# HSU-ANT/gstpeaq

Measured on AMD Instinct MI355X. Metric: 2048-sample stereo ref/test frame-pairs/sec (basic PEAQ, ear model -> MOVs -> ODG); ODG delta vs CPU ref, higher is better.
Workload: dtype f64

## Files before the change

### gstpeaq_amd/capi.py

```python
import ctypes as C
import os
import subprocess
from pathlib import Path

import numpy as np

PKG = Path(__file__).resolve().parent
ROOT = PKG.parent

MOV_NAMES_BASIC = ["BandwidthRefB", "BandwidthTestB", "TotalNMRB", "WinModDiff1B", "ADBB", "EHSB",
                   "AvgModDiff1B", "AvgModDiff2B", "RmsNoiseLoudB", "MFPDB", "RelDistFramesB"]
MOV_NAMES_ADVANCED = ["RmsModDiffA", "RmsNoiseLoudAsymA", "SegmentalNMRB", "EHSB", "AvgLinDistA"]

RESULT_DOUBLES = 16
RECORD_DOUBLES = 576


class Settings(C.Structure):
    _fields_ = [("swap_mod_patts_for_noise_loudness_movs", C.c_int), ("center_ehs_correlation_window", C.c_int),
                ("ehs_subtract_dc_before_window", C.c_int), ("use_floor_for_steps_above_threshold", C.c_int),
                ("clamp_movs", C.c_int), ("swap_slope_filter_coefficients", C.c_int)]


class PeaqError(RuntimeError):
# ... 197 lines not shown
        L.peaq_batch_measure_gain.argtypes = [vp, C.c_int, C.c_int, vp, C.c_size_t, u32p, vp, C.c_size_t, u32p, u32p, C.c_int,
                                              C.c_double, vp, vp]
        L.peaq_gain_workspace_bytes.restype = C.c_size_t
        L.peaq_gain_workspace_bytes.argtypes = [C.c_int, C.c_int, C.c_uint32]
        L.peaq_batch_cut_scaled.argtypes = [vp, C.c_int, C.c_int, vp, C.c_size_t, u32p, u32p, vp, vp, C.c_size_t, vp]
        L.peaq_run_pair_matched.argtypes = [vp, C.c_int, C.c_int, C.c_double, C.c_uint32, C.c_uint32, C.c_int, C.c_double, fp,
                                            C.c_size_t, fp, C.c_size_t, C.POINTER(Delay), C.POINTER(Gain), dp]
        L.peaq_batch_run_host_matched.argtypes = [vp, C.c_int, C.c_double, C.POINTER(Feed), C.c_int, C.c_double, C.c_size_t,
                                                  C.POINTER(HostSignal), C.c_size_t, C.POINTER(HostTest), dp, C.POINTER(Delay),
                                                  C.POINTER(Gain)]
        L.peaq_feed_matched_workspace_bytes.restype = C.c_size_t
        L.peaq_feed_matched_workspace_bytes.argtypes = [C.POINTER(Feed), C.c_int, C.c_int, C.c_size_t, C.c_size_t, C.c_uint64]
    L.peaq_batch_last_timing.argtypes = [vp, C.POINTER(_Timing)]
    if hasattr(L, "peaq_calibrate"):
        L.peaq_calibrate.argtypes = [vp, C.c_int, C.POINTER(_Calibration)]
        L.peaq_batch_last_clock.argtypes = [vp, dp]
    L.peaq_synth_fill.argtypes = [vp, C.c_uint32, C.c_int, C.c_int, C.c_uint32, C.c_size_t, vp, vp, vp]
    L.peaq_debug_frontend.argtypes = [vp, C.c_int, C.c_int, C.c_double, vp, vp, C.c_uint32, C.c_uint32,
                                      C.c_int, dp]
    L.peaq_debug_filterbank.argtypes = [vp, C.c_int, C.c_double, vp, vp, C.c_uint32, C.c_uint32, C.c_int, C.c_int, dp]
    if hasattr(L, "peaq_debug_wave"):
        L.peaq_debug_wave.argtypes = [vp, C.c_char_p, C.c_size_t, C.c_int, dp, C.c_int, dp, C.c_int, dp]
        L.peaq_debug_common_tables.argtypes = [dp, dp]
    ip = C.POINTER(C.c_int)
    L.peaq_broker_create.argtypes = [vp, C.c_int, C.c_int, C.c_double, C.c_int, C.POINTER(vp)]
    L.peaq_broker_create_multi.argtypes = [C.POINTER(C.c_int), C.c_int, C.c_int, C.c_int, C.c_double, C.c_int, vp, C.c_int,
                                           C.POINTER(vp)]
    L.peaq_broker_devices.argtypes = [vp]
    if hasattr(L, "peaq_debug_broker_fail_shard"):
        L.peaq_debug_broker_fail_shard.argtypes = [vp, C.c_int, C.c_char_p]
    L.peaq_broker_stats_size.argtypes = []
    L.peaq_broker_stats_size.restype = C.c_size_t
    L.peaq_broker_destroy.argtypes = [vp]
    L.peaq_broker_destroy.restype = None
    L.peaq_broker_open.argtypes = [vp, ip]
    L.peaq_broker_close.argtypes = [vp, C.c_int]
    L.peaq_broker_push.argtypes = [vp, C.c_int, C.c_int, fp, C.c_size_t]
    L.peaq_broker_flush.argtypes = [vp, C.c_int]
    L.peaq_broker_tick.argtypes = [vp, C.POINTER(C.c_uint)]
    L.peaq_broker_results.argtypes = [vp, C.c_int, dp]
    L.peaq_broker_start.argtypes = [vp, C.c_uint]
    L.peaq_broker_stop.argtypes = [vp]
    L.peaq_broker_stats.argtypes = [vp, C.POINTER(_BrokerStats)]
    _LIB = L
    return L

# ... 979 lines not shown
```

### gstpeaq_amd/csrc/peaq_debug_wave.hip

```cpp
#include "peaq_host.h"
#include "peaq_wave.h"

using namespace peaq;

namespace {

constexpr int kWgThreads = 256;

enum WaveOp : int {
  OP_LOG_POS, OP_LOG_POS_SK, OP_LOG_NONNEG, OP_LOG_NONNEG_SK, OP_LOG_TAB, OP_LOG_TAB_NONNEG,
  OP_EXP_FAST, OP_EXP_FAST_SK, OP_EXP_TAB, OP_SQRT_POS, OP_RSQRT_POS, OP_DIV_FAST, OP_POW_POS, OP_POW_TAB,
  OP_POW_LOGTAB, OP_LOG_NONNEG_N5, OP_EXP_FAST_N5,
  OP_WAVE_SUM, OP_WAVE_MAX, OP_WAVE_SUM2, OP_WAVE_SUM4, OP_WAVE_PREFIX_SUM, OP_WAVE_SUFFIX_GEOMETRIC,
  OP_WAVE_PREFIX_GEOMETRIC, OP_WAVE_PREFIX_GEOMETRIC_Z, OP_WAVE_PREFIX_GEOMETRIC_F32, OP_ROWS_TRANSPOSE4,
  OP_LANE_BELOW, OP_LANE_ABOVE, OP_READ_LANE_0, OP_READ_LANE_63, OP_DFT4, OP_DFT8, OP_DFT16, OP_COUNT
};

struct OpInfo {
  const char* name;
  int planes_in, planes_out, n_params;
};
const OpInfo kOps[OP_COUNT] = {
    {"log_pos", 1, 1, 0},
    {"log_pos_sk", 1, 1, 0},
// ... 174 lines not shown
                                  " planes and returns " + std::to_string(info.planes_out));
  if (n_params != info.n_params || (n_params > 0 && !params))
    return fail(PEAQ_ERR_ARG, std::string("peaq_debug_wave: ") + op + " takes " + std::to_string(info.n_params) + " parameters");
  if (!c || !in || !out) return fail(PEAQ_ERR_ARG, "peaq_debug_wave: NULL argument");
  if (n > ((size_t)1 << 26)) return fail(PEAQ_ERR_ARG, "peaq_debug_wave: more than 2^26 elements per plane");
  if (n == 0) return PEAQ_OK;
  HIP_TRY(hipSetDevice(c->device));
  const size_t n_pad = (n + kWgThreads - 1) / kWgThreads * kWgThreads;
  DevBuf d_in, d_out;
  HIP_TRY(d_in.reserve((size_t)planes_in * n_pad * sizeof(double)));
  HIP_TRY(d_out.reserve((size_t)planes_out * n_pad * sizeof(double)));
  HIP_TRY(hipMemset(d_in.p, 0, (size_t)planes_in * n_pad * sizeof(double)));
  HIP_TRY(hipMemset(d_out.p, 0, (size_t)planes_out * n_pad * sizeof(double)));
  for (int p = 0; p < planes_in; ++p)
    HIP_TRY(hipMemcpy(d_in.as<double>() + (size_t)p * n_pad, in + (size_t)p * n, n * sizeof(double), hipMemcpyHostToDevice));
  HIP_TRY(hipDeviceSynchronize());
  HIP_TRY(launch_one<0>(which, d_in.as<double>(), d_out.as<double>(), n_pad, n_params ? params[0] : 0., c->d_common));
  HIP_TRY(hipDeviceSynchronize());
  for (int p = 0; p < planes_out; ++p)
    HIP_TRY(hipMemcpy(out + (size_t)p * n, d_out.as<double>() + (size_t)p * n_pad, n * sizeof(double), hipMemcpyDeviceToHost));
  return PEAQ_OK;
}

extern "C" int peaq_debug_common_tables(double* log_tab, double* exp_tab) {
  if (!log_tab || !exp_tab) return fail(PEAQ_ERR_ARG, "peaq_debug_common_tables: NULL argument");
  auto ct = std::make_unique<CommonTables>();
  build_common_tables(*ct);
  std::memcpy(log_tab, ct->log_tab, sizeof ct->log_tab);
  std::memcpy(exp_tab, ct->exp_tab, sizeof ct->exp_tab);
  return PEAQ_OK;
}
```

### gstpeaq_amd/csrc/peaq_frontend.hip

```cpp
#include <hip/hip_runtime.h>

#include "peaq_device.h"
#include "peaq_kernels.h"
#include <type_traits>

#include "peaq_wave.h"

namespace peaq {

#ifndef PEAQ_FE_PREFETCH_ITEMS
#define PEAQ_FE_PREFETCH_ITEMS 64
#endif
constexpr int kPrefetchItems = PEAQ_FE_PREFETCH_ITEMS;
constexpr int kUnitDoubles = 1288;
constexpr int kOffPw = 0;
constexpr int kOffScratch = 776;
constexpr int kPwLen = 776;
constexpr int kOffLogTab = 2 * kUnitDoubles;
constexpr int kLogTabDoubles = 2 * kLogTabEntries + 2;
constexpr int kLdsDoubles = 2 * kUnitDoubles + 2 * kLogTabDoubles;
#ifndef PEAQ_FE_WAVES
#define PEAQ_FE_WAVES 3
#endif
constexpr int kWavesPerSimd = PEAQ_FE_WAVES;

__device__ constexpr double kW32re[16] = {1., 0.98078528040323044913, 0.92387953251128675613, 0.83146961230254523708,
                                          0.70710678118654752440, 0.55557023301960222474, 0.38268343236508977173,
                                          0.19509032201612826785, 0., -0.19509032201612826785, -0.38268343236508977173,
                                          -0.55557023301960222474, -0.70710678118654752440, -0.83146961230254523708,
                                          -0.92387953251128675613, -0.98078528040323044913};
__device__ constexpr double kW32im[16] = {-0., -0.19509032201612826785, -0.38268343236508977173, -0.55557023301960222474,
                                          -0.70710678118654752440, -0.83146961230254523708, -0.92387953251128675613,
                                          -0.98078528040323044913, -1., -0.98078528040323044913, -0.92387953251128675613,
                                          -0.83146961230254523708, -0.70710678118654752440, -0.55557023301960222474,
                                          -0.38268343236508977173, -0.19509032201612826785};

__device__ __forceinline__ int pad16(int i) { return i + (i >> 4); }

__device__ __forceinline__ cplx tw_lane(const CommonTables* __restrict__ ct, int e, int lane) {
  const double2 v = *reinterpret_cast<const double2*>(ct->tw_lane[e][lane]);
  return {v.x, v.y};
}
__device__ __forceinline__ cplx csqr(cplx a) { return {a.re * a.re - a.im * a.im, 2. * (a.re * a.im)}; }

template <typename WR, typename RD>
__device__ __forceinline__ void exchange16(cplx (&z)[16], double* buf, WR wr, RD rd) {
#pragma unroll
  for (int r = 0; r < 16; ++r) buf[pad16(wr(r))] = z[r].re;
  wave_lds_fence();
#pragma unroll
  for (int r = 0; r < 16; ++r) z[r].re = buf[pad16(rd(r))];
  wave_lds_fence();
#pragma unroll
  for (int r = 0; r < 16; ++r) buf[pad16(wr(r))] = z[r].im;
  wave_lds_fence();
#pragma unroll
  for (int r = 0; r < 16; ++r) z[r].im = buf[pad16(rd(r))];
  wave_lds_fence();
}

__device__ __forceinline__ void frame_power_spectrum(cplx (&z)[16], double (&p)[16], double* unit, int lane,
                                                     const CommonTables* __restrict__ ct,
                                                     double level_factor) {
  dft16(z);
// ... 31 lines not shown
        z[4 * a2 + g] = z[4 * g + a2];
        z[4 * g + a2] = t;
      }
#else
    const int k = lane & 15, j = (lane - k) * 16 + k;
    exchange16(z, unit, [&](int r) { return j + 16 * r; },
               [&](int s) { return lane + 64 * (s & 3) + 256 * (s >> 2); });
#endif
  }
  {
    constexpr double c1 = 0.92387953251128673848, s1 = 0.38268343236508977173, c2 = 0.70710678118654752440;
    const cplx wb = tw_lane(ct, 1, lane);
#pragma unroll
    for (int m = 0; m < 4; ++m) {
      const cplx w1 = m == 0 ? wb : m == 1 ? cmul(wb, {c1, -s1}) : m == 2 ? cmul(wb, {c2, -c2}) : cmul(wb, {s1, -c1});
      const cplx w2 = csqr(w1), w3 = cmul(w2, w1);
      z[m + 4] = cmul(z[m + 4], w1);
      z[m + 8] = cmul(z[m + 8], w2);
      z[m + 12] = cmul(z[m + 12], w3);
      dft4(z[m], z[m + 4], z[m + 8], z[m + 12]);
    }
  }
  wave_lds_fence();
  const cplx wl = tw_lane(ct, 0, lane);
  const int partner = (64 - lane) & 63;
  const double lf4 = 0.25 * level_factor;
#pragma unroll
  for (int q = 0; q < 8; ++q) {
    const int k = lane + 64 * q;
    cplx zm = {__shfl(z[15 - q].re, partner, 64), __shfl(z[15 - q].im, partner, 64)};
    if (lane == 0) zm = z[(16 - q) & 15];
    const cplx e2 = {z[q].re + zm.re, z[q].im - zm.im};
    const cplx o2 = {z[q].im + zm.im, zm.re - z[q].re};
    const cplx wq = {kW32re[q], kW32im[q]};
    const cplx t = cmul(q == 0 ? wl : cmul(wl, wq), o2);
    const cplx xp = cadd(e2, t), xm = csub(e2, t);
    p[q] = (xp.re * xp.re + xp.im * xp.im) * lf4;
    double pm = (xm.re * xm.re + xm.im * xm.im) * lf4;
    int km = 1024 - k;
    if (q == 0 && lane == 0) {
      pm = (z[8].re * z[8].re + z[8].im * z[8].im) * level_factor;
      km = 512;
    }
    p[8 + q] = pm;
    const double2 ew = *reinterpret_cast<const double2*>(ct->ear_w2_pair[q][lane]);
    unit[kOffPw + k] = p[q] * ew.x;
    if (km < kPwLen) unit[kOffPw + km] = pm * ew.y;
  }
  wave_lds_fence();
}

__device__ __forceinline__ int spec_bin(int s, int lane) {
  if (s < 8) return lane + 64 * s;
// ... 93 lines not shown
  do {                                                                                 \
    const unsigned long long now_ = __builtin_readcyclecounter();                      \
    if (a.prof && lane == 0 && (blockIdx.x & 127) == 5) atomicAdd(a.prof + sig * 16 + (i), now_ - prof_t_); \
    prof_t_ = __builtin_readcyclecounter();                                            \
  } while (0)
#else
#define FE_MARK(i) do { } while (0)
#endif

template <int NB>
__global__ __launch_bounds__(128, kWavesPerSimd)
#ifdef PEAQ_FE_NUM_VGPR
__attribute__((amdgpu_num_vgpr(PEAQ_FE_NUM_VGPR)))
#endif
void frontend_kernel(FrontendArgs a) {
  extern __shared__ double lds[];
  __builtin_amdgcn_s_setprio(3);
#ifndef PEAQ_FE_LAZY_KERNARGS
  asm volatile("" ::"s"(a.ref), "s"(a.test), "s"(a.pair_stride), "s"(a.n_ref), "s"(a.n_test), "s"(a.n_uniform_ref),
               "s"(a.n_uniform_test), "s"(a.n_frames), "s"(a.n_frames_uniform), "s"(a.frame_origin), "s"(a.off_ref),
               "s"(a.off_test), "s"(a.channels), "s"(a.frame0), "s"(a.frames_per_launch), "s"(a.fpl_magic), "s"(a.common),
               "s"(a.records), "s"(a.pair_frame0), "s"(gridDim.x));
#endif
  const int lane = threadIdx.x & 63;
  const int sig = __builtin_amdgcn_readfirstlane(threadIdx.x >> 6);
#ifdef PEAQ_FE_PROFILE
  unsigned long long prof_t_ = __builtin_readcyclecounter();
  if (a.prof && lane == 0 && (blockIdx.x & 127) == 5) atomicAdd(a.prof + 32 + sig, 1ull);
#endif
  double* unit = lds + sig * kUnitDoubles;
  double* scratch = unit + kOffScratch;
  const CommonTables* __restrict__ ct = a.common;
  const BandTables* __restrict__ bt = a.bands;

  auto decode = [&](unsigned it, unsigned& pair_, unsigned& fl_) {
    const unsigned t = it >> (a.channels - 1);
    pair_ = a.frames_per_launch == 1 ? t : __umulhi(t, a.fpl_magic);
    fl_ = t - pair_ * a.frames_per_launch;
    return (int)(it & (unsigned)(a.channels - 1));
  };
  const unsigned item = xcd_remap(blockIdx.x, gridDim.x);
  unsigned pair, fl;
  const int chan = decode(item, pair, fl);
  FE_MARK(15);
  const unsigned n_ref = a.n_ref ? a.n_ref[pair] : a.n_uniform_ref;
  const unsigned n_test = a.n_test ? a.n_test[pair] : a.n_uniform_test;
  unsigned frame, frame_origin;
  if (a.pair_frame0) {
    if (fl >= a.pair_nframes[pair]) return;
    frame_origin = a.pair_frame0[pair];
    frame = frame_origin + fl;
  } else {
    frame = a.frame0 + fl;
    frame_origin = a.frame_origin;
// ... 3 lines not shown
  const size_t pair_off = (size_t)pair * a.pair_stride * a.channels;
  FrameSrc src_ref, src_test;
  {
    const long long s0 = (long long)(frame - frame_origin) * kHop;
    src_ref.set(a.ref + pair_off, s0 + a.off_ref, (long long)n_ref, a.channels, chan);
    src_test.set(a.test + pair_off, s0 + a.off_test, (long long)n_test, a.channels, chan);
  }
  const FrameSrc& src = sig ? src_test : src_ref;
  double* __restrict__ rec =
      a.records + ((size_t)(pair * a.frames_per_launch + fl) * a.channels + chan) * kRecDoubles;
  constexpr double kHannA = 0.81649658092772603273;
  constexpr double kHannC[16] = {1.0, 0.923806101034885660186, 0.7068354246185547448714, 0.3821516543455241229047,
                                 -0.0007673650086148258012924, -0.3835694472988822502431, -0.7079202261619581075015,
                                 -0.9243926006499437062869, -0.9999988223018871071366, -0.9232174254904238786877,
                                 -0.7057489581976599840459, -0.3807329612736016723471, 0.002302093218395832312485,
                                 0.3849863367942118830771, 0.7090033602727326108775, 0.9249769229541590372578};
  constexpr double kHannS[16] = {0.0, 0.382860663545790020567, 0.7073780336597309217442, 0.92409962292005024589,
                                 0.99999970557542843387, 0.923512035167290059731, 0.7062923993579444458354,
                                 0.3814424201155840173045, -0.001534729565367423810065, -0.3842780051874341062575,
                                 -0.7084620018059667117941, -0.924685034052046356158, -0.9999973501798961346679,
                                 -0.9229222721777677728372, -0.705205101457706221079, -0.3800232782373413192215};
  const double2 hl0 = *reinterpret_cast<const double2*>(&ct->hann_lane[lane][0]);
  const double2 hl1 = *reinterpret_cast<const double2*>(&ct->hann_lane[lane][2]);
  double* ltab = lds + kOffLogTab + sig * kLogTabDoubles;
  FE_MARK(13);
  cplx z[16];
  float amax = 0.f;
  double energy = 0., hop = 0.;
  {
    const int voff = src.lane_offset(lane);
#pragma unroll
    for (int r = 0; r < 16; ++r) {
      const int n = lane + 64 * r;
      float x0, x1;
      src.load2(r, voff, x0, x1);
      const double w0 = fma(hl0.y, kHannS[r], fma(-hl0.x, kHannC[r], kHannA));
      const double w1 = fma(hl1.y, kHannS[r], fma(-hl1.x, kHannC[r], kHannA));
      z[r] = {w0 * (double)x0, w1 * (double)x1};
      if (r >= 8) {
        energy += (double)(x0 * x0);
        energy += (double)(x1 * x1);
      } else if (sig == 0) {
        hop += (double)(x0 * x0);
        hop += (double)(x1 * x1);
      } else {
        float r0, r1;
        src_ref.load2(r, voff, r0, r1);
// ... 5 lines not shown
  }
  float pf_keep = 0.f;
  if (chan == 0 && !a.pair_frame0) {
    const unsigned it2 = item + kPrefetchItems;
    if (it2 < gridDim.x) {
      unsigned pair2, fl2;
      decode(it2, pair2, fl2);
      const unsigned n2 = sig ? (a.n_test ? a.n_test[pair2] : a.n_uniform_test) : (a.n_ref ? a.n_ref[pair2] : a.n_uniform_ref);
      const long long s2 = (long long)(a.frame0 + fl2 - a.frame_origin) * kHop + (fl2 == 0 ? 0 : kHop);
      FrameSrc pf;
      pf.set((sig ? a.test : a.ref) + (size_t)pair2 * a.pair_stride * a.channels, s2 + (sig ? a.off_test : a.off_ref),
             (long long)n2, a.channels, 0);
      pf_keep = __uint_as_float(__builtin_amdgcn_raw_buffer_load_b32(pf.rs, lane * 128, 0, 0));
      if (fl2 == 0 && a.channels == 2)
        pf_keep += __uint_as_float(__builtin_amdgcn_raw_buffer_load_b32(pf.rs, (64 + lane) * 128, 0, 0));
    }
  }

  __builtin_amdgcn_s_setprio(0);
#ifdef PEAQ_FE_PROFILE
  asm volatile("s_waitcnt vmcnt(0)" ::: "memory");
#endif
  FE_MARK(14);
  wave_sum2(hop, energy, hop, energy);
  if (lane == 0) rec[sig ? kRecNoiseE : kRecSigE] = hop;
  const int energy_flag = energy >= 8000. / (32768. * 32768.);

  int above = 0;
  if (sig == 0) {
    if (__any((double)amax >= 200. / 32768 + 1e-6)) {
      above = 1;
    } else {
      float* ax = reinterpret_cast<float*>(unit);
      int lane_q = lane;
      asm volatile("" : "+v"(lane_q));
      const int voff_q = src.lane_offset(lane_q);
#pragma unroll
      for (int r = 0; r < 16; ++r) {
        const int n = lane_q + 64 * r;
        float x0, x1;
        src.load2(r, voff_q, x0, x1);
        reinterpret_cast<float2*>(ax)[n] = make_float2(fabsf(x0), fabsf(x1));
      }
      wave_lds_fence();
      above = boundary_detect(ax, kFrame, lane);
      wave_lds_fence();
    }
  }

  if (lane == 0)
    rec[sig ? kRecFlagsTest : kRecFlagsRef] = (double)(above | (energy_flag << 1));

  FE_MARK(0);
  double pspec[16];
  frame_power_spectrum(z, pspec, unit, lane, ct, a.level_factor);

  const int gb1 = lane < (NB + 1) / 2 ? lane : 0, gb2 = lane < (NB + 1) / 2 ? NB - 1 - lane : 0;
  const BandEdge edge1 = load_band_edge(bt, gb1), edge2 = load_band_edge(bt, gb2);
  {
    const double2 t0 = *reinterpret_cast<const double2*>(ct->log_tab[lane]);
    const double2 t1 = *reinterpret_cast<const double2*>(ct->log_tab[64 + lane]);
    const double2 t2 = *reinterpret_cast<const double2*>(ct->log_tab[128]);
    reinterpret_cast<double2*>(ltab)[lane] = t0;
    reinterpret_cast<double2*>(ltab)[64 + lane] = t1;
    if (lane == 0) reinterpret_cast<double2*>(ltab)[128] = t2;
    wave_lds_fence();
  }
  FE_MARK(1);
  constexpr bool kAdvanced = NB == 55;
  int bw_ref = 0, bw_test = 0;
  double* xch = lds + kOffLogTab + 2 * kLogTabEntries;
  double thr = 0.;
  auto top_bin = [&](double level, int limit, bool or_equal) {
    int best = 0;
#pragma unroll
    for (int q = 0; q < 8; ++q) {
      unsigned long long m = __ballot(or_equal ? pspec[q] >= level : pspec[q] > level);
      const int nl = limit - 64 * q;
      m &= nl >= 64 ? ~0ull : nl <= 0 ? 0ull : (1ull << nl) - 1ull;
      if (m) best = max(best, 64 * q + 64 - __builtin_clzll(m));
    }
#pragma unroll
    for (int q = 0; q < 8; ++q) {
      unsigned long long m = __ballot(or_equal ? pspec[8 + q] >= level : pspec[8 + q] > level);
      if (q == 0) {
        if ((m & 1ull) && 512 < limit) best = max(best, 513);
        m &= ~1ull;
      }
      const int lo = 1024 - 64 * q - limit + 1;
      m &= lo >= 64 ? 0ull : lo <= 0 ? ~0ull : ~0ull << lo;
      if (m) best = max(best, 1024 - 64 * q - __builtin_ctzll(m) + 1);
    }
    return best;
  };
  if (!kAdvanced && sig == 1) {
    if (lane >= 1) thr = pspec[8];
    if (lane <= 39) thr = fmax(thr, pspec[9]);
    thr = wave_max(thr);
    if (lane == 0) xch[0] = thr;
  }

  FE_MARK(2);
  const double* pw_ref = lds + kOffPw;
  double* pw_test = lds + kUnitDoubles + kOffPw;
  double* sa = lds + kOffScratch;
  double* sb = lds + kUnitDoubles + kOffScratch;
  int* adv_flag = reinterpret_cast<int*>(lds + kOffLogTab + kLogTabDoubles + 2 * kLogTabEntries);
  auto wait_flag = [&](int i) {
    while (__builtin_amdgcn_readfirstlane(*(volatile int*)(adv_flag + i)) == 0) __builtin_amdgcn_s_sleep(1);
    wave_lds_fence();
  };
  if constexpr (kAdvanced) {
    if (sig == 0 && lane == 0) {
      adv_flag[0] = 0;
      adv_flag[1] = 0;
    }
    __syncthreads();
    if (sig == 1) {
#pragma unroll
      for (int j = 0; j < 8; ++j) {
        const int k = lane + 64 * j;
        const double fr = pw_ref[k], ft = pw_test[k];
        sb[k] = (fr == 0. && ft == 0.) ? 0. : FE_LOG_NONNEG(ft / fr, ltab);
      }
      FE_MARK(8);
      wave_lds_fence();
      {
        constexpr int kSteps = (kPwLen + 63) / 64;
        double r[kSteps], t[kSteps];
#pragma unroll
        for (int i = 0; i < kSteps; ++i) {
          const int k = lane + 64 * i < kPwLen ? lane + 64 * i : 0;
          r[i] = pw_ref[k];
          t[i] = pw_test[k];
        }
        wave_lds_fence();
#pragma unroll
        for (int i = 0; i < kSteps; ++i)
          if (lane + 64 * i < kPwLen) pw_test[lane + 64 * i] = r[i] - 2 * sqrt_pos(r[i] * t[i]) + t[i];
      }
      wave_lds_fence();
      if (lane == 0) adv_flag[1] = 1;
      FE_MARK(10);
    }
  }
  if (!kAdvanced || sig == 0) {
    const double* pw = unit + kOffPw;
    constexpr int kZeroSlot = kOffScratch + 400 - kOffPw;
    if (lane == 0) scratch[400] = 0.;
    wave_lds_fence();
    double* ppx = scratch + 256;
    const int b0 = 2 * lane;
    double c_noise[2], c_lnauc[2], c_gil[2];
#pragma unroll
    for (int s2 = 0; s2 < 2; ++s2) {
      const int b = b0 + s2 < NB ? b0 + s2 : 0;
      c_noise[s2] = bt->internal_noise[b];
      c_lnauc[s2] = bt->ln_aUC[b];
      c_gil[s2] = bt->gIL[b];
    }
    if (lane < (NB + 1) / 2) {
      const int b1 = lane, b2 = NB - 1 - lane;
      ppx[b1] = group_band(edge1, pw, kZeroSlot);
      if (b2 != b1) ppx[b2] = group_band(edge2, pw, kZeroSlot);
    }
    wave_lds_fence();
    if (kAdvanced && lane == 0) adv_flag[0] = 1;
    FE_MARK(3);
    constexpr int kLanes = (NB - 1) / 2;
    double ene[2], ae[2], far[2], back2[2];
#pragma unroll
    for (int s = 0; s < 2; ++s) {
      const int b = b0 + s;
      if (b < NB) {
        const double pp = ppx[b] + c_noise[s];
        const double ln_pp = FE_LOG(pp, ltab);
        const double ln_a = c_lnauc[s] + bt->dz02 * ln_pp;
        const double t = exp_fast(0.2 * ln_a), t2 = t * t;
        const double a_uce = t2 * t2 * t;
        const double g_iu = div_fast(1. - exp_fast((double)(NB - b) * ln_a), 1. - a_uce);
        ae[s] = t2;
        ene[s] = exp_fast(0.4 * (ln_pp - FE_LOG(c_gil[s] + g_iu - 1., ltab)));
        {
          double pw = 1., sq = t2;
#pragma unroll
          for (int e = 2 * kLanes - s; e; e >>= 1) {
            if (e & 1) pw *= sq;
            if (e >> 1) sq *= sq;
          }
          far[s] = ene[s] * pw;
        }
        const double t4 = t2 * t2;
        back2[s] = t4 > 1e-290 ? div_fast(1., t4) : 0.;
      } else {
        ae[s] = 0.;
        ene[s] = 0.;
        far[s] = 0.;
        back2[s] = 0.;
// ... 19 lines not shown
    FE_MARK(5);
    double dn0, dn1;
    {
      const double al = bt->aLe;
      const double v = wave_suffix_geometric(ene[0] + al * ene[1], al * al, lane);
      const double nxt = lane_above(v);
      dn0 = v;
      dn1 = ene[1] + al * nxt;
    }
    double root[2];
#pragma unroll
    for (int s = 0; s < 2; ++s) {
      const double e2 = (s ? dn1 : dn0) + (s ? up1 : up0);
      root[s] = b0 + s < NB ? sqrt_pos(sqrt_pos(e2)) : 0.;
    }
    if (b0 < kBandStride)
      *reinterpret_cast<double2*>(rec + (sig ? kRecRootTest : kRecRootRef) + b0) = make_double2(root[0], root[1]);

  }
  FE_MARK(6);
  if constexpr (kAdvanced) {
    if (sig == 0) {
      const BandEdge e1 = load_band_edge(bt, gb1), e2 = load_band_edge(bt, gb2);
      if (lane == 0) xch[0] = 0.;
      wait_flag(1);
      const int zero_at = (int)(xch - pw_test);
      if (lane < (NB + 1) / 2) {
        const int b1 = lane, b2 = NB - 1 - lane;
        rec[kRecNoise + b1] = group_band(e1, pw_test, zero_at);
        if (b2 != b1) rec[kRecNoise + b2] = group_band(e2, pw_test, zero_at);
      } else if (lane < (NB + 1) / 2 + kBandStride - NB) {
        rec[kRecNoise + NB + lane - (NB + 1) / 2] = 0.;
      }
      if (lane == 0) {
        rec[kRecBwRef] = 0.;
        rec[kRecBwTest] = 0.;
      }
    } else {
      wait_flag(0);
    }
    FE_MARK(7);
  } else {
    __syncthreads();
    FE_MARK(7);
    if (sig == 0) {
      bw_ref = top_bin(10. * xch[0], 921, false);
      if (lane == 0) xch[1] = (double)bw_ref;
    }
  }

  if constexpr (!kAdvanced) {
    double* dlog = sa;
#ifndef PEAQ_FE_RATIOS_REF
#define PEAQ_FE_RATIOS_REF 3
#endif
    constexpr int kRefRatios = PEAQ_FE_RATIOS_REF;
#pragma unroll
    for (int j = 0; j < 8 - kRefRatios; ++j) {
      if (sig == 0 && j >= kRefRatios) break;
      const int k = (sig == 0 ? 0 : 64 * kRefRatios) + lane + 64 * j;
      const double fr = pw_ref[k], ft = pw_test[k];
      dlog[k] = (fr == 0. && ft == 0.) ? 0. : FE_LOG_NONNEG(ft / fr, ltab);
    }
  }
  if constexpr (!kAdvanced) {
    FE_MARK(8);
    __syncthreads();
    FE_MARK(9);
  }
  if (!kAdvanced && sig == 1) {
    bw_ref = (int)xch[1];
    if (bw_ref > 346) bw_test = top_bin(3.16227766016838 * thr, bw_ref, true);
  }

  if (!kAdvanced && sig == 1) {
    wave_lds_fence();
    {
      constexpr int kSteps = (kPwLen + 63) / 64;
      double r[kSteps], t[kSteps];
#pragma unroll
      for (int i = 0; i < kSteps; ++i) {
        const int k = lane + 64 * i < kPwLen ? lane + 64 * i : 0;
        r[i] = pw_ref[k];
        t[i] = pw_test[k];
      }
      wave_lds_fence();
#pragma unroll
      for (int i = 0; i < kSteps; ++i)
        if (lane + 64 * i < kPwLen) pw_test[lane + 64 * i] = r[i] - 2 * sqrt_pos(r[i] * t[i]) + t[i];
      if (lane == 0) lds[kOffPw] = 0.;
    }
    wave_lds_fence();
    if (lane < (NB + 1) / 2) {
      const int b1 = lane, b2 = NB - 1 - lane;
      rec[kRecNoise + b1] = group_band(edge1, pw_test, kOffPw - kUnitDoubles);
      if (b2 != b1) rec[kRecNoise + b2] = group_band(edge2, pw_test, kOffPw - kUnitDoubles);
    } else if (lane < (NB + 1) / 2 + kBandStride - NB) {
      rec[kRecNoise + NB + lane - (NB + 1) / 2] = 0.;
    }
    if (lane == 0) {
      rec[kRecBwRef] = (double)bw_ref;
      rec[kRecBwTest] = (double)bw_test;
    }
    FE_MARK(10);
  } else if (kAdvanced ? sig == 1 : sig == 0) {
    double* const sa = kAdvanced ? lds + kOffPw : lds + kOffScratch;
    cplx u[8];
    double g[4], run_in;
    {
      const double* d = kAdvanced ? sb : sa;
#pragma unroll
      for (int r = 0; r < 8; ++r) {
        const double v = d[lane + 64 * r];
        u[r] = {r < 4 ? v : 0., v};
      }
      double tot = 0.;
#pragma unroll
      for (int t = 0; t < 4; ++t) {
        const int j = 4 * lane + t;
        const double hi = d[j + 256], lo = d[j];
        g[t] = hi * hi - lo * lo;
        tot += g[t];
      }
      run_in = wave_prefix_sum(tot, lane) - tot;
    }
    wave_lds_fence();
    auto exchange8 = [&](auto wr, auto swz) {
#pragma unroll
      for (int r = 0; r < 8; ++r) {
        const int i = swz(wr(r));
        sa[i] = u[r].re;
        sb[i] = u[r].im;
      }
      wave_lds_fence();
#pragma unroll
      for (int r = 0; r < 8; ++r) {
        const int i = swz(lane + 64 * r);
        u[r] = {sa[i], sb[i]};
      }
      wave_lds_fence();
    };
    auto twiddle8 = [&](cplx w1) {
      cplx w[8];
      w[1] = w1;
      w[2] = csqr(w[1]);
      w[4] = csqr(w[2]);
      w[3] = cmul(w[1], w[2]);
      w[5] = cmul(w[4], w[1]);
      w[6] = cmul(w[4], w[2]);
      w[7] = cmul(w[4], w[3]);
#pragma unroll
      for (int r = 1; r < 8; ++r) u[r] = cmul(u[r], w[r]);
    };
    dft8(u);
    exchange8([&](int r) { return 8 * lane + r; }, [](int i) { return i ^ ((i >> 4) & 7); });
    {
      const int k = lane & 7;
      twiddle8(tw_lane(ct, 4, lane));
      dft8(u);
      const int j = (lane - k) * 8 + k;
      exchange8([&](int r) { return j + 8 * r; }, [](int i) { return i ^ (((i >> 6) & 1) << 3); });
    }
    const cplx w512 = tw_lane(ct, 3, lane);
    twiddle8(w512);
    dft8(u);
    FE_MARK(10);
    const int partner = (64 - lane) & 63;
    cplx cc[4];
    double c256 = 0.;
#pragma unroll
    for (int r = 0; r < 4; ++r) {
      cplx zm = {__shfl(u[7 - r].re, partner, 64), __shfl(u[7 - r].im, partner, 64)};
      if (lane == 0) zm = u[(8 - r) & 7];
      const cplx a2 = {u[r].re + zm.re, u[r].im - zm.im};
      const cplx b2 = {u[r].im + zm.im, zm.re - u[r].re};
      cc[r] = {b2.re * a2.re + b2.im * a2.im, b2.im * a2.re - b2.re * a2.im};
    }
    if (lane == 0) c256 = (2. * u[4].re) * (2. * u[4].im);
    cplx v[4];
#pragma unroll
    for (int r = 0; r < 4; ++r) {
      cplx cm = {__shfl(cc[3 - r].re, partner, 64), __shfl(cc[3 - r].im, partner, 64)};
      if (lane == 0) cm = r == 0 ? cplx{c256, 0.} : cc[4 - r];
      const cplx e = {cc[r].re + cm.re, cc[r].im - cm.im};
      const cplx od = {cc[r].re - cm.re, cc[r].im + cm.im};
      constexpr double c8 = 0.70710678118654752440;
      const cplx wkf = r == 0 ? w512 : r == 1 ? cmul(w512, {c8, -c8}) : r == 2 ? cmul_mi(w512) : cmul(w512, {-c8, -c8});
      const cplx o = cmul(od, {wkf.re, -wkf.im});
      v[r] = {e.re - o.im, -(e.im + o.re)};
    }
    wave_lds_fence();
    double2* xb = reinterpret_cast<double2*>(sa);
    auto fft256 = [&](cplx (&w)[4]) {
#pragma unroll
      for (int pass = 0; pass < 4; ++pass) {
        const int p = 1 << (2 * pass);
        const int k = lane & (p - 1);
        if (pass > 0) {
          if (pass < 3) {
#pragma unroll
            for (int r = 0; r < 4; ++r) {
              const double2 x = xb[lane + 64 * r];
              w[r] = {x.x, x.y};
            }
          }
// ... 50 lines not shown
#pragma unroll
    for (int m = 0; m < 4; ++m) w4[m] = {(c[m] - cavg) * win[lane + 64 * m], 0.};
    wave_lds_fence();
    fft256(w4);
    if (!a.cfg.ehs_dc_before_window && lane == 0) w4[0].re = 0.;
    const double s0 = w4[0].re * w4[0].re + w4[0].im * w4[0].im;
    const double s1 = w4[1].re * w4[1].re + w4[1].im * w4[1].im;
    const double s2 = w4[2].re * w4[2].re + w4[2].im * w4[2].im;
    const double s0_up = lane_below(s0), s1_up = lane_below(s1);
    const double s0_last = read_lane<63>(s0), s1_last = read_lane<63>(s1);
    const double prev0 = s0_up;
    const double prev1 = lane == 0 ? s0_last : s1_up;
    double best = 0.;
    if (lane >= 1 && s0 > prev0) best = s0;
    if (s1 > prev1 && s1 > best) best = s1;
    if (lane == 0 && s2 > s1_last && s2 > best) best = s2;
    best = wave_max(best);
    if (lane == 0) rec[kRecEhs] = best;
    FE_MARK(12);
  }
  if (pf_keep == 123456.789f) rec[kRecScalars + 15] = 1.;
}

hipError_t launch_frontend(int bands, const FrontendArgs& a, unsigned n_pairs, hipStream_t stream) {
  const unsigned grid = n_pairs * a.frames_per_launch * a.channels;
  if (grid == 0) return hipSuccess;
  if ((unsigned long long)n_pairs * a.frames_per_launch * a.channels >= (1ull << 26)) return hipErrorInvalidValue;
  FrontendArgs args = a;
  args.fpl_magic = (unsigned)(((1ull << 32) + a.frames_per_launch - 1) / a.frames_per_launch);
  if (a.frames_per_launch > 1) {
    const unsigned long long err = (unsigned long long)args.fpl_magic * a.frames_per_launch - (1ull << 32);
    const unsigned long long t_max = (unsigned long long)n_pairs * a.frames_per_launch - 1;
    if (err && t_max >= ((1ull << 32) + err - 1) / err) return hipErrorInvalidValue;
  }
#ifndef PEAQ_FE_LDS_PAD
#define PEAQ_FE_LDS_PAD 0
#endif
  const size_t lds = kLdsDoubles * sizeof(double) + PEAQ_FE_LDS_PAD;
  if (bands == 109)
    hipLaunchKernelGGL(frontend_kernel<109>, dim3(grid), dim3(128), lds, stream, args);
  else if (bands == 55)
    hipLaunchKernelGGL(frontend_kernel<55>, dim3(grid), dim3(128), lds, stream, args);
  else
    return hipErrorInvalidValue;
  return hipGetLastError();
}

}
```

### gstpeaq_amd/csrc/peaq_kernels.h

```cpp
#pragma once
#include <hip/hip_runtime.h>

#include "peaq_device.h"

namespace peaq {

struct FrontendArgs {
  const float* ref;
  const float* test;
  size_t pair_stride;
  const uint32_t* n_ref;
  const uint32_t* n_test;
  uint32_t n_uniform_ref;
  uint32_t n_uniform_test;
  const uint32_t* n_frames;
  uint32_t n_frames_uniform;
  unsigned frame_origin;
  long long off_ref, off_test;
  int channels;
  unsigned frame0;
  unsigned frames_per_launch;
  unsigned fpl_magic;
  double level_factor;
  const CommonTables* common;
  const BandTables* bands;
  double* records;
  const uint32_t* pair_frame0;
  const uint32_t* pair_nframes;
  unsigned long long* prof;
  Settings cfg;
};
hipError_t launch_frontend(int bands, const FrontendArgs& a, unsigned n_pairs, hipStream_t stream);
inline unsigned max_frames_per_launch(unsigned n_pairs) {
  unsigned long long d = 65535;
  while (d > 1 && (unsigned long long)(n_pairs ? n_pairs : 1) * d * d > (1ull << 32)) d >>= 1;
  return (unsigned)d;
}

struct PointArgs {
  PointSnap* snap;
  const uint32_t* n_ref;
  const uint32_t* n_test;
  uint32_t n_uniform;
  uint32_t interval;
  int n_points;
};

constexpr uint32_t kTraceAbove = 1u, kTraceModOpen = 2u, kTraceLoudOpen = 4u, kTraceFlush = 8u;
struct FrameTrace {
  double ch[2][6];
  double p_detect, steps;
  uint32_t flags, frame;
  double reserved;
};
struct BlockTrace {
// ... 106 lines not shown
```

### include/peaq_amd.h

```cpp
#ifndef PEAQ_AMD_H
#define PEAQ_AMD_H

#include <stddef.h>
#include <stdint.h>

#ifdef __cplusplus
extern "C" {
#endif

#define PEAQ_OK            0
#define PEAQ_ERR_ARG      -1
#define PEAQ_ERR_DEVICE   -2
#define PEAQ_ERR_NOMEM    -3
#define PEAQ_ERR_STATE    -4

#define PEAQ_MOVS_BASIC     11
#define PEAQ_MOVS_ADVANCED   5

typedef struct {
  double movs[PEAQ_MOVS_BASIC];
  double di;
  double odg;
  double totalsnr;
  double frames;
// ... 282 lines not shown
int peaq_debug_frontend (peaq_ctx *ctx, int bands, int channels, double playback_level_db,
                         const float *d_ref, const float *d_test, uint32_t n_ref, uint32_t n_test,
                         int n_frames, double *host_out);

#define PEAQ_DEBUG_FB_RECORD_DOUBLES 168
int peaq_debug_filterbank (peaq_ctx *ctx, int channels, double playback_level_db,
                           const float *d_ref, const float *d_test, uint32_t n_ref, uint32_t n_test,
                           int n_blocks, int blocks_per_launch, double *host_out);

#define PEAQ_DEBUG_BACKEND_DOUBLES 912
int peaq_debug_backend (peaq_ctx *ctx, int channels, int n_frames, const double *host_records,
                        double *host_out, peaq_result *result);

double peaq_debug_fb_tables_selfcheck (void);

#define PEAQ_DEBUG_ADV_BLOCK_DOUBLES 8
int peaq_debug_backend_advanced (peaq_ctx *ctx, int channels, int n_blocks, const double *fb_records,
                                 int n_frames, const double *fft_records, double *out_blocks,
                                 double *out_frames, peaq_result *result);

int peaq_debug_wave (peaq_ctx *ctx, const char *op, size_t n, int planes_in, const double *in,
                     int n_params, const double *params, int planes_out, double *out);

int peaq_debug_common_tables (double *log_tab , double *exp_tab );

#define PEAQ_DEBUG_STREAM_WINDOW_FIELDS 5
int peaq_debug_stream_plan (int advanced, unsigned max_frames, unsigned max_blocks, int drain_every_push,
                            size_t n_pushes, const int *pad, const uint64_t *n_samples, size_t max_windows,
                            uint64_t *windows, size_t *n_windows);

#ifdef __cplusplus
}
#endif
#endif
```

Before: 28.16 million.

## Shrink frontend LDS footprint and replace barriers with workgroup flags

Reorganizes the frontend kernel's LDS layout so each wave's unit is just the FFT buffer, with log ratios, band sums and EHS buffers aliased into spare tail space, and a single shared log table. This brings LDS under a budget of eight workgroups per CU and raises the waves-per-SIMD default from 3 to 4, aiming at higher occupancy. The threshold/bandwidth handoff between the two signal waves now uses release/acquire LDS flags instead of __syncthreads, and cross-lane shuffles are replaced with ds_bpermute-based reads. The aliasing is intricate and correctness relies on the flag ordering and the static_asserts about overlap.

Result: no change. 28.06 million (-0.4%).

```diff
diff --git a/gstpeaq_amd/capi.py b/gstpeaq_amd/capi.py
--- a/gstpeaq_amd/capi.py
+++ b/gstpeaq_amd/capi.py
@@ -243,6 +243,9 @@
     if hasattr(L, "peaq_debug_wave"):
         L.peaq_debug_wave.argtypes = [vp, C.c_char_p, C.c_size_t, C.c_int, dp, C.c_int, dp, C.c_int, dp]
         L.peaq_debug_common_tables.argtypes = [dp, dp]
+    if hasattr(L, "peaq_debug_frontend_lds_bytes"):
+        L.peaq_debug_frontend_lds_bytes.argtypes = []
+        L.peaq_debug_frontend_lds_bytes.restype = C.c_size_t
     ip = C.POINTER(C.c_int)
     L.peaq_broker_create.argtypes = [vp, C.c_int, C.c_int, C.c_double, C.c_int, C.POINTER(vp)]
     L.peaq_broker_create_multi.argtypes = [C.POINTER(C.c_int), C.c_int, C.c_int, C.c_int, C.c_double, C.c_int, vp, C.c_int,
diff --git a/gstpeaq_amd/csrc/peaq_debug_wave.hip b/gstpeaq_amd/csrc/peaq_debug_wave.hip
--- a/gstpeaq_amd/csrc/peaq_debug_wave.hip
+++ b/gstpeaq_amd/csrc/peaq_debug_wave.hip
@@ -220,6 +220,8 @@
   return PEAQ_OK;
 }
 
+extern "C" size_t peaq_debug_frontend_lds_bytes(void) { return frontend_lds_bytes(); }
+
 extern "C" int peaq_debug_common_tables(double* log_tab, double* exp_tab) {
   if (!log_tab || !exp_tab) return fail(PEAQ_ERR_ARG, "peaq_debug_common_tables: NULL argument");
   auto ct = std::make_unique<CommonTables>();
diff --git a/gstpeaq_amd/csrc/peaq_frontend.hip b/gstpeaq_amd/csrc/peaq_frontend.hip
--- a/gstpeaq_amd/csrc/peaq_frontend.hip
+++ b/gstpeaq_amd/csrc/peaq_frontend.hip
@@ -12,17 +12,44 @@
 #define PEAQ_FE_PREFETCH_ITEMS 64
 #endif
 constexpr int kPrefetchItems = PEAQ_FE_PREFETCH_ITEMS;
-constexpr int kUnitDoubles = 1288;
+constexpr int kFftBufDoubles = 1024 + 1024 / 16;
+constexpr int kUnitDoubles = kFftBufDoubles;
 constexpr int kOffPw = 0;
-constexpr int kOffScratch = 776;
 constexpr int kPwLen = 776;
+constexpr int kOffTail = kOffPw + kPwLen;
+constexpr int kTailDoubles = kUnitDoubles - kOffTail;
+static_assert(kTailDoubles >= 256, "half of the log ratios fits behind a spectrum");
+constexpr int kOffPpx = kOffTail;
+constexpr int kOffBandZero = kOffPpx + 128;
+constexpr int kOffDlogHi = kOffTail;
+constexpr int kOffDlogLo = kUnitDoubles + kOffTail;
+constexpr int kOffEhsA = 0, kOffEhsB = 512;
 constexpr int kOffLogTab = 2 * kUnitDoubles;
-constexpr int kLogTabDoubles = 2 * kLogTabEntries + 2;
-constexpr int kLdsDoubles = 2 * kUnitDoubles + 2 * kLogTabDoubles;
+constexpr int kLogTabDoubles = 2 * kLogTabEntries;
+constexpr int kOffXch = kOffLogTab + kLogTabDoubles;
+constexpr int kLdsDoubles = kOffXch + 4;
+constexpr int kFlagThr = 0;
+constexpr int kFlagBwRef = 1;
+constexpr int kFlagRefSpecFree = 2;
+constexpr int kFlagNoise = 3;
 #ifndef PEAQ_FE_WAVES
-#define PEAQ_FE_WAVES 3
+#define PEAQ_FE_WAVES 4
 #endif
 constexpr int kWavesPerSimd = PEAQ_FE_WAVES;
+constexpr int kLdsBudgetBytes = 160 * 1024 / 8;
+static_assert(kLdsDoubles * sizeof(double) <= kLdsBudgetBytes, "LDS: eight workgroups per CU");
+static_assert(kUnitDoubles >= kFftBufDoubles, "the first FFT exchange runs in both units at the same time");
+static_assert(kUnitDoubles * sizeof(double) >= kFrame * sizeof(float), "the quiet-frame path stages |x| in the unit");
+static_assert(kOffBandZero < kUnitDoubles && kOffPpx >= kOffPw + kPwLen, "band sums beside the spectrum they add up");
+static_assert(kOffDlogHi >= kOffPw + kPwLen && kOffDlogHi + 256 <= kUnitDoubles, "log ratios beside the reference spectrum");
+static_assert(kOffDlogLo >= kUnitDoubles + kOffPw + kPwLen && kOffDlogLo + 256 <= 2 * kUnitDoubles,
+              "log ratios beside the test unit's (noise) spectrum");
+static_assert(kOffEhsA + 512 <= kOffEhsB && kOffEhsB + 512 <= kUnitDoubles,
+              "EHS exchange buffers: disjoint, inside the reference unit (away from d[0..255] and the noise spectrum)");
+static_assert(kOffLogTab >= 2 * kUnitDoubles && kOffXch >= kOffLogTab + 2 * kLogTabEntries,
+              "table and flag words alias nothing the FFT exchanges write");
+static_assert(kOffPpx % 2 == 0 && kUnitDoubles % 2 == 0 && kOffLogTab % 2 == 0 && kOffXch % 2 == 0 && kOffEhsB % 2 == 0,
+              "16-byte accesses");
 
 __device__ constexpr double kW32re[16] = {1., 0.98078528040323044913, 0.92387953251128675613, 0.83146961230254523708,
                                           0.70710678118654752440, 0.55557023301960222474, 0.38268343236508977173,
@@ -40,6 +67,12 @@
 __device__ __forceinline__ cplx tw_lane(const CommonTables* __restrict__ ct, int e, int lane) {
   const double2 v = *reinterpret_cast<const double2*>(ct->tw_lane[e][lane]);
   return {v.x, v.y};
+}
+__device__ __forceinline__ double lane_read(double v, int idx4) {
+  const long long b = __double_as_longlong(v);
+  const unsigned lo = (unsigned)__builtin_amdgcn_ds_bpermute(idx4, (int)(unsigned)b);
+  const unsigned hi = (unsigned)__builtin_amdgcn_ds_bpermute(idx4, (int)(unsigned)(b >> 32));
+  return __longlong_as_double((long long)(((unsigned long long)hi << 32) | lo));
 }
 __device__ __forceinline__ cplx csqr(cplx a) { return {a.re * a.re - a.im * a.im, 2. * (a.re * a.im)}; }
 
@@ -117,13 +150,17 @@
     }
   }
   wave_lds_fence();
+#pragma unroll
+  for (int r = 0; r < 16; r += 4)
+    asm volatile("" : "+v"(z[r].re), "+v"(z[r].im), "+v"(z[r + 1].re), "+v"(z[r + 1].im), "+v"(z[r + 2].re), "+v"(z[r + 2].im),
+                 "+v"(z[r + 3].re), "+v"(z[r + 3].im));
   const cplx wl = tw_lane(ct, 0, lane);
-  const int partner = (64 - lane) & 63;
+  const int partner4 = ((64 - lane) & 63) * 4;
   const double lf4 = 0.25 * level_factor;
 #pragma unroll
   for (int q = 0; q < 8; ++q) {
     const int k = lane + 64 * q;
-    cplx zm = {__shfl(z[15 - q].re, partner, 64), __shfl(z[15 - q].im, partner, 64)};
+    cplx zm = {lane_read(z[15 - q].re, partner4), lane_read(z[15 - q].im, partner4)};
     if (lane == 0) zm = z[(16 - q) & 15];
     const cplx e2 = {z[q].re + zm.re, z[q].im - zm.im};
     const cplx o2 = {z[q].im + zm.im, zm.re - z[q].re};
@@ -263,14 +300,28 @@
                "s"(a.off_test), "s"(a.channels), "s"(a.frame0), "s"(a.frames_per_launch), "s"(a.fpl_magic), "s"(a.common),
                "s"(a.records), "s"(a.pair_frame0), "s"(gridDim.x));
 #endif
-  const int lane = threadIdx.x & 63;
+  int lane = threadIdx.x & 63;
   const int sig = __builtin_amdgcn_readfirstlane(threadIdx.x >> 6);
 #ifdef PEAQ_FE_PROFILE
   unsigned long long prof_t_ = __builtin_readcyclecounter();
   if (a.prof && lane == 0 && (blockIdx.x & 127) == 5) atomicAdd(a.prof + 32 + sig, 1ull);
 #endif
   double* unit = lds + sig * kUnitDoubles;
-  double* scratch = unit + kOffScratch;
+  double* xch = lds + kOffXch;
+  int* flags = reinterpret_cast<int*>(lds + kOffXch + 2);
+  auto raise_flag = [&](int i, int value) {
+    __builtin_amdgcn_fence(__ATOMIC_RELEASE, "workgroup");
+    if (lane == 0) __hip_atomic_store(flags + i, value, __ATOMIC_RELEASE, __HIP_MEMORY_SCOPE_WORKGROUP);
+  };
+  auto wait_flag = [&](int i) {
+    int v;
+    while ((v = __builtin_amdgcn_readfirstlane(
+                __hip_atomic_load(flags + i, __ATOMIC_ACQUIRE, __HIP_MEMORY_SCOPE_WORKGROUP))) == 0)
+      __builtin_amdgcn_s_sleep(1);
+    __builtin_amdgcn_fence(__ATOMIC_ACQUIRE, "workgroup");
+    return v;
+  };
+  if (sig == 0 && lane == 0) *reinterpret_cast<int4*>(flags) = make_int4(0, 0, 0, 0);
   const CommonTables* __restrict__ ct = a.common;
   const BandTables* __restrict__ bt = a.bands;
 
@@ -320,7 +371,7 @@
                                  -0.9229222721777677728372, -0.705205101457706221079, -0.3800232782373413192215};
   const double2 hl0 = *reinterpret_cast<const double2*>(&ct->hann_lane[lane][0]);
   const double2 hl1 = *reinterpret_cast<const double2*>(&ct->hann_lane[lane][2]);
-  double* ltab = lds + kOffLogTab + sig * kLogTabDoubles;
+  double* ltab = lds + kOffLogTab;
   FE_MARK(13);
   cplx z[16];
   float amax = 0.f;
@@ -372,6 +423,7 @@
   asm volatile("s_waitcnt vmcnt(0)" ::: "memory");
 #endif
   FE_MARK(14);
+  if constexpr (NB != 55) __syncthreads();
   wave_sum2(hop, energy, hop, energy);
   if (lane == 0) rec[sig ? kRecNoiseE : kRecSigE] = hop;
   const int energy_flag = energy >= 8000. / (32768. * 32768.);
@@ -403,24 +455,24 @@
 
   FE_MARK(0);
   double pspec[16];
+  asm volatile("" : "+v"(lane));
   frame_power_spectrum(z, pspec, unit, lane, ct, a.level_factor);
 
-  const int gb1 = lane < (NB + 1) / 2 ? lane : 0, gb2 = lane < (NB + 1) / 2 ? NB - 1 - lane : 0;
-  const BandEdge edge1 = load_band_edge(bt, gb1), edge2 = load_band_edge(bt, gb2);
-  {
-    const double2 t0 = *reinterpret_cast<const double2*>(ct->log_tab[lane]);
-    const double2 t1 = *reinterpret_cast<const double2*>(ct->log_tab[64 + lane]);
-    const double2 t2 = *reinterpret_cast<const double2*>(ct->log_tab[128]);
-    reinterpret_cast<double2*>(ltab)[lane] = t0;
-    reinterpret_cast<double2*>(ltab)[64 + lane] = t1;
-    if (lane == 0) reinterpret_cast<double2*>(ltab)[128] = t2;
-    wave_lds_fence();
-  }
+  constexpr bool kAdvanced = NB == 55;
+  asm volatile("" : "+v"(lane));
+  lane &= 63;
+  double2 lt0 = {}, lt1 = {}, lt2 = {};
+  if (sig == 0) {
+    lt0 = *reinterpret_cast<const double2*>(ct->log_tab[lane]);
+    lt1 = *reinterpret_cast<const double2*>(ct->log_tab[64 + lane]);
+    lt2 = *reinterpret_cast<const double2*>(ct->log_tab[128]);
+  }
+  auto store_log_table = [&]() {
+    reinterpret_cast<double2*>(ltab)[lane] = lt0;
+    reinterpret_cast<double2*>(ltab)[64 + lane] = lt1;
+    if (lane == 0) reinterpret_cast<double2*>(ltab)[128] = lt2;
+  };
   FE_MARK(1);
-  constexpr bool kAdvanced = NB == 55;
-  int bw_ref = 0, bw_test = 0;
-  double* xch = lds + kOffLogTab + 2 * kLogTabEntries;
-  double thr = 0.;
   auto top_bin = [&](double level, int limit, bool or_equal) {
     int best = 0;
 #pragma unroll
@@ -443,35 +495,50 @@
     }
     return best;
   };
-  if (!kAdvanced && sig == 1) {
+  if constexpr (kAdvanced) {
+    if (sig == 0) store_log_table();
+  } else if (sig == 1) {
+    double thr = 0.;
     if (lane >= 1) thr = pspec[8];
     if (lane <= 39) thr = fmax(thr, pspec[9]);
     thr = wave_max(thr);
     if (lane == 0) xch[0] = thr;
-  }
-
-  FE_MARK(2);
+    raise_flag(kFlagThr, 1);
+    FE_MARK(2);
+    const int bw_ref = wait_flag(kFlagBwRef) - 1;
+    int bw_test = 0;
+    if (bw_ref > 346) bw_test = top_bin(3.16227766016838 * thr, bw_ref, true);
+    if (lane == 0) {
+      rec[kRecBwRef] = (double)bw_ref;
+      rec[kRecBwTest] = (double)bw_test;
+    }
+  } else {
+    store_log_table();
+    wait_flag(kFlagThr);
+    const int bw_ref = top_bin(10. * xch[0], 921, false);
+    raise_flag(kFlagBwRef, bw_ref + 1);
+    FE_MARK(2);
+  }
+  const int gb1 = lane < (NB + 1) / 2 ? lane : 0, gb2 = lane < (NB + 1) / 2 ? NB - 1 - lane : 0;
+  const BandEdge edge1 = load_band_edge(bt, gb1), edge2 = load_band_edge(bt, gb2);
+
   const double* pw_ref = lds + kOffPw;
   double* pw_test = lds + kUnitDoubles + kOffPw;
-  double* sa = lds + kOffScratch;
-  double* sb = lds + kUnitDoubles + kOffScratch;
-  int* adv_flag = reinterpret_cast<int*>(lds + kOffLogTab + kLogTabDoubles + 2 * kLogTabEntries);
-  auto wait_flag = [&](int i) {
-    while (__builtin_amdgcn_readfirstlane(*(volatile int*)(adv_flag + i)) == 0) __builtin_amdgcn_s_sleep(1);
-    wave_lds_fence();
-  };
+  double* dlo = lds + kOffDlogLo;
+  double* dhi = lds + kOffDlogHi;
+  double dhi_keep[4] = {};
   if constexpr (kAdvanced) {
-    if (sig == 0 && lane == 0) {
-      adv_flag[0] = 0;
-      adv_flag[1] = 0;
-    }
     __syncthreads();
     if (sig == 1) {
 #pragma unroll
       for (int j = 0; j < 8; ++j) {
         const int k = lane + 64 * j;
         const double fr = pw_ref[k], ft = pw_test[k];
-        sb[k] = (fr == 0. && ft == 0.) ? 0. : FE_LOG_NONNEG(ft / fr, ltab);
+        const double d = (fr == 0. && ft == 0.) ? 0. : FE_LOG_NONNEG(ft / fr, ltab);
+        if (j < 4)
+          dlo[k] = d;
+        else
+          dhi_keep[j - 4] = d;
       }
       FE_MARK(8);
       wave_lds_fence();
@@ -490,16 +557,16 @@
           if (lane + 64 * i < kPwLen) pw_test[lane + 64 * i] = r[i] - 2 * sqrt_pos(r[i] * t[i]) + t[i];
       }
       wave_lds_fence();
-      if (lane == 0) adv_flag[1] = 1;
+      raise_flag(kFlagNoise, 1);
       FE_MARK(10);
     }
   }
   if (!kAdvanced || sig == 0) {
     const double* pw = unit + kOffPw;
-    constexpr int kZeroSlot = kOffScratch + 400 - kOffPw;
-    if (lane == 0) scratch[400] = 0.;
+    constexpr int kZeroSlot = kOffBandZero - kOffPw;
+    if (lane == 0) unit[kOffBandZero] = 0.;
     wave_lds_fence();
-    double* ppx = scratch + 256;
+    double* ppx = unit + kOffPpx;
     const int b0 = 2 * lane;
     double c_noise[2], c_lnauc[2], c_gil[2];
 #pragma unroll
@@ -515,7 +582,9 @@
       if (b2 != b1) ppx[b2] = group_band(edge2, pw, kZeroSlot);
     }
     wave_lds_fence();
-    if (kAdvanced && lane == 0) adv_flag[0] = 1;
+    const double2 ppv = reinterpret_cast<const double2*>(ppx)[lane];
+    wave_lds_fence();
+    if constexpr (kAdvanced) raise_flag(kFlagRefSpecFree, 1);
     FE_MARK(3);
     constexpr int kLanes = (NB - 1) / 2;
     double ene[2], ae[2], far[2], back2[2];
@@ -523,7 +592,7 @@
     for (int s = 0; s < 2; ++s) {
       const int b = b0 + s;
       if (b < NB) {
-        const double pp = ppx[b] + c_noise[s];
+        const double pp = (s ? ppv.y : ppv.x) + c_noise[s];
         const double ln_pp = FE_LOG(pp, ltab);
         const double ln_a = c_lnauc[s] + bt->dz02 * ln_pp;
         const double t = exp_fast(0.2 * ln_a), t2 = t * t;
@@ -589,9 +658,9 @@
   if constexpr (kAdvanced) {
     if (sig == 0) {
       const BandEdge e1 = load_band_edge(bt, gb1), e2 = load_band_edge(bt, gb2);
-      if (lane == 0) xch[0] = 0.;
-      wait_flag(1);
-      const int zero_at = (int)(xch - pw_test);
+      if (lane == 0) xch[1] = 0.;
+      wait_flag(kFlagNoise);
+      constexpr int zero_at = kOffXch + 1 - (kUnitDoubles + kOffPw);
       if (lane < (NB + 1) / 2) {
         const int b1 = lane, b2 = NB - 1 - lane;
         rec[kRecNoise + b1] = group_band(e1, pw_test, zero_at);
@@ -604,30 +673,33 @@
         rec[kRecBwTest] = 0.;
       }
     } else {
-      wait_flag(0);
+      wait_flag(kFlagRefSpecFree);
+#pragma unroll
+      for (int j = 0; j < 4; ++j) dhi[lane + 64 * j] = dhi_keep[j];
+      wave_lds_fence();
     }
     FE_MARK(7);
   } else {
     __syncthreads();
     FE_MARK(7);
-    if (sig == 0) {
-      bw_ref = top_bin(10. * xch[0], 921, false);
-      if (lane == 0) xch[1] = (double)bw_ref;
-    }
   }
 
   if constexpr (!kAdvanced) {
-    double* dlog = sa;
 #ifndef PEAQ_FE_RATIOS_REF
 #define PEAQ_FE_RATIOS_REF 3
 #endif
     constexpr int kRefRatios = PEAQ_FE_RATIOS_REF;
+    static_assert(kRefRatios >= 1 && kRefRatios <= 4, "the reference wave takes 1..4 of the 8 log ratios per lane");
 #pragma unroll
     for (int j = 0; j < 8 - kRefRatios; ++j) {
       if (sig == 0 && j >= kRefRatios) break;
       const int k = (sig == 0 ? 0 : 64 * kRefRatios) + lane + 64 * j;
       const double fr = pw_ref[k], ft = pw_test[k];
-      dlog[k] = (fr == 0. && ft == 0.) ? 0. : FE_LOG_NONNEG(ft / fr, ltab);
+      const double d = (fr == 0. && ft == 0.) ? 0. : FE_LOG_NONNEG(ft / fr, ltab);
+      if (sig == 0 || j < 4 - kRefRatios)
+        dlo[k] = d;
+      else
+        dhi[k - 256] = d;
     }
   }
   if constexpr (!kAdvanced) {
@@ -635,11 +707,6 @@
     __syncthreads();
     FE_MARK(9);
   }
-  if (!kAdvanced && sig == 1) {
-    bw_ref = (int)xch[1];
-    if (bw_ref > 346) bw_test = top_bin(3.16227766016838 * thr, bw_ref, true);
-  }
-
   if (!kAdvanced && sig == 1) {
     wave_lds_fence();
     {
@@ -652,46 +719,45 @@
         t[i] = pw_test[k];
       }
       wave_lds_fence();
+      raise_flag(kFlagRefSpecFree, 1);
 #pragma unroll
       for (int i = 0; i < kSteps; ++i)
         if (lane + 64 * i < kPwLen) pw_test[lane + 64 * i] = r[i] - 2 * sqrt_pos(r[i] * t[i]) + t[i];
-      if (lane == 0) lds[kOffPw] = 0.;
+      if (lane == 0) xch[1] = 0.;
     }
     wave_lds_fence();
+    constexpr int zero_at = kOffXch + 1 - (kUnitDoubles + kOffPw);
     if (lane < (NB + 1) / 2) {
       const int b1 = lane, b2 = NB - 1 - lane;
-      rec[kRecNoise + b1] = group_band(edge1, pw_test, kOffPw - kUnitDoubles);
-      if (b2 != b1) rec[kRecNoise + b2] = group_band(edge2, pw_test, kOffPw - kUnitDoubles);
+      rec[kRecNoise + b1] = group_band(edge1, pw_test, zero_at);
+      if (b2 != b1) rec[kRecNoise + b2] = group_band(edge2, pw_test, zero_at);
     } else if (lane < (NB + 1) / 2 + kBandStride - NB) {
       rec[kRecNoise + NB + lane - (NB + 1) / 2] = 0.;
     }
-    if (lane == 0) {
-      rec[kRecBwRef] = (double)bw_ref;
-      rec[kRecBwTest] = (double)bw_test;
-    }
     FE_MARK(10);
   } else if (kAdvanced ? sig == 1 : sig == 0) {
-    double* const sa = kAdvanced ? lds + kOffPw : lds + kOffScratch;
+    double* const sa = lds + kOffEhsA;
+    double* const sb = lds + kOffEhsB;
     cplx u[8];
     double g[4], run_in;
     {
-      const double* d = kAdvanced ? sb : sa;
 #pragma unroll
       for (int r = 0; r < 8; ++r) {
-        const double v = d[lane + 64 * r];
+        const double v = r < 4 ? dlo[lane + 64 * r] : dhi[lane + 64 * (r - 4)];
         u[r] = {r < 4 ? v : 0., v};
       }
       double tot = 0.;
 #pragma unroll
       for (int t = 0; t < 4; ++t) {
         const int j = 4 * lane + t;
-        const double hi = d[j + 256], lo = d[j];
+        const double hi = dhi[j], lo = dlo[j];
         g[t] = hi * hi - lo * lo;
         tot += g[t];
       }
       run_in = wave_prefix_sum(tot, lane) - tot;
     }
     wave_lds_fence();
+    if constexpr (!kAdvanced) wait_flag(kFlagRefSpecFree);
     auto exchange8 = [&](auto wr, auto swz) {
 #pragma unroll
       for (int r = 0; r < 8; ++r) {
@@ -732,12 +798,12 @@
     twiddle8(w512);
     dft8(u);
     FE_MARK(10);
-    const int partner = (64 - lane) & 63;
+    const int partner4 = ((64 - lane) & 63) * 4;
     cplx cc[4];
     double c256 = 0.;
 #pragma unroll
     for (int r = 0; r < 4; ++r) {
-      cplx zm = {__shfl(u[7 - r].re, partner, 64), __shfl(u[7 - r].im, partner, 64)};
+      cplx zm = {lane_read(u[7 - r].re, partner4), lane_read(u[7 - r].im, partner4)};
       if (lane == 0) zm = u[(8 - r) & 7];
       const cplx a2 = {u[r].re + zm.re, u[r].im - zm.im};
       const cplx b2 = {u[r].im + zm.im, zm.re - u[r].re};
@@ -747,7 +813,7 @@
     cplx v[4];
 #pragma unroll
     for (int r = 0; r < 4; ++r) {
-      cplx cm = {__shfl(cc[3 - r].re, partner, 64), __shfl(cc[3 - r].im, partner, 64)};
+      cplx cm = {lane_read(cc[3 - r].re, partner4), lane_read(cc[3 - r].im, partner4)};
       if (lane == 0) cm = r == 0 ? cplx{c256, 0.} : cc[4 - r];
       const cplx e = {cc[r].re + cm.re, cc[r].im - cm.im};
       const cplx od = {cc[r].re - cm.re, cc[r].im + cm.im};
@@ -844,6 +910,11 @@
   if (pf_keep == 123456.789f) rec[kRecScalars + 15] = 1.;
 }
 
+#ifndef PEAQ_FE_LDS_PAD
+#define PEAQ_FE_LDS_PAD 0
+#endif
+size_t frontend_lds_bytes() { return kLdsDoubles * sizeof(double) + PEAQ_FE_LDS_PAD; }
+
 hipError_t launch_frontend(int bands, const FrontendArgs& a, unsigned n_pairs, hipStream_t stream) {
   const unsigned grid = n_pairs * a.frames_per_launch * a.channels;
   if (grid == 0) return hipSuccess;
@@ -855,10 +926,7 @@
     const unsigned long long t_max = (unsigned long long)n_pairs * a.frames_per_launch - 1;
     if (err && t_max >= ((1ull << 32) + err - 1) / err) return hipErrorInvalidValue;
   }
-#ifndef PEAQ_FE_LDS_PAD
-#define PEAQ_FE_LDS_PAD 0
-#endif
-  const size_t lds = kLdsDoubles * sizeof(double) + PEAQ_FE_LDS_PAD;
+  const size_t lds = frontend_lds_bytes();
   if (bands == 109)
     hipLaunchKernelGGL(frontend_kernel<109>, dim3(grid), dim3(128), lds, stream, args);
   else if (bands == 55)
diff --git a/gstpeaq_amd/csrc/peaq_kernels.h b/gstpeaq_amd/csrc/peaq_kernels.h
--- a/gstpeaq_amd/csrc/peaq_kernels.h
+++ b/gstpeaq_amd/csrc/peaq_kernels.h
@@ -31,6 +31,7 @@
   Settings cfg;
 };
 hipError_t launch_frontend(int bands, const FrontendArgs& a, unsigned n_pairs, hipStream_t stream);
+size_t frontend_lds_bytes();
 inline unsigned max_frames_per_launch(unsigned n_pairs) {
   unsigned long long d = 65535;
   while (d > 1 && (unsigned long long)(n_pairs ? n_pairs : 1) * d * d > (1ull << 32)) d >>= 1;
diff --git a/include/peaq_amd.h b/include/peaq_amd.h
--- a/include/peaq_amd.h
+++ b/include/peaq_amd.h
@@ -328,6 +328,8 @@
 int peaq_debug_wave (peaq_ctx *ctx, const char *op, size_t n, int planes_in, const double *in,
                      int n_params, const double *params, int planes_out, double *out);
 
+size_t peaq_debug_frontend_lds_bytes (void);
+
 int peaq_debug_common_tables (double *log_tab , double *exp_tab );
 
 #define PEAQ_DEBUG_STREAM_WINDOW_FIELDS 5
```
